# nie-lang/StabStitch2

Hardware: AMD Instinct MI355X
Metric: stitched frames/sec, 720p 2-view (StabStitch++ inference hot path) (higher is better)
Workload: dtype f32; 1 GPU; configs[2]: 720x1280 2-view, 32-frame clip per step per GPU, 7-frame SmoothWarp sliding window, warp NORMAL / fusion AVERAGE, synthetic checkpoints; parallelism=streams1

## Files before the change

__graft_entry__.py:

```python
import os
import subprocess
import sys

ROOT = os.path.dirname(os.path.abspath(__file__))
if ROOT not in sys.path:
    sys.path.insert(0, ROOT)


def build():
    subprocess.run(['bash', os.path.join(ROOT, 'stabstitch2_amd', 'csrc', 'build.sh')], check=True)
    subprocess.run(['bash', os.path.join(ROOT, 'stabstitch2_amd', 'csrc', 'build.sh'), 'tuning'], check=True)
    import re
    from stabstitch2_amd import _hip
    lib = _hip.lib()
    hdr = open(os.path.join(ROOT, 'include', 'stabstitch_hip.h')).read()
    declared = sorted(set(re.findall(r'\b(ss_[a-z0-9_]+)\s*\(', hdr)))
    missing = [n for n in declared if not hasattr(lib, n)]
    if missing:
        raise RuntimeError('libstabstitch_hip.so lacks symbols declared in the header: %s' % missing)
    if sorted(_hip.SIGNATURES) != declared:
        raise RuntimeError('ctypes table and header disagree: %s' % sorted(set(_hip.SIGNATURES) ^ set(declared)))
    from stabstitch2_amd import _blend
    blib = _blend.lib()
    bhdr = open(os.path.join(ROOT, 'include', 'stabstitch_blend.h')).read()
    bdeclared = sorted(set(re.findall(r'\bSSB_API[^;]*?\b(ssb_[a-z0-9_]+)\s*\(', bhdr)))
    missing = [n for n in bdeclared if not hasattr(blib, n)]
    if missing:
        raise RuntimeError('libstabstitch_blend.so lacks symbols declared in the header: %s' % missing)
    if sorted(_blend.SIGNATURES) != bdeclared:
        raise RuntimeError('ctypes table and header disagree: %s' % sorted(set(_blend.SIGNATURES) ^ set(bdeclared)))
    from stabstitch2_amd import _seam
    slib = _seam.lib()
    shdr = open(os.path.join(ROOT, 'include', 'stabstitch_seam.h')).read()
    sdeclared = sorted(set(re.findall(r'\bSSM_API[^;]*?\b(ssm_[a-z0-9_]+)\s*\(', shdr)))
    missing = [n for n in sdeclared if not hasattr(slib, n)]
    if missing:
        raise RuntimeError('libstabstitch_seam.so lacks symbols declared in the header: %s' % missing)
    if sorted(_seam.SIGNATURES) != sdeclared:
        raise RuntimeError('ctypes table and header disagree: %s' % sorted(set(_seam.SIGNATURES) ^ set(sdeclared)))
    from stabstitch2_amd import _mbwarp
    wlib = _mbwarp.lib()
    whdr = open(os.path.join(ROOT, 'include', 'stabstitch_mbwarp.h')).read()
    wdeclared = sorted(set(re.findall(r'\bSSW_API[^;]*?\b(ssw_[a-z0-9_]+)\s*\(', whdr)))
    missing = [n for n in wdeclared if not hasattr(wlib, n)]
    if missing:
        raise RuntimeError('libstabstitch_mbwarp.so lacks symbols declared in the header: %s' % missing)
    if sorted(_mbwarp.SIGNATURES) != wdeclared:
        raise RuntimeError('ctypes table and header disagree: %s' % sorted(set(_mbwarp.SIGNATURES) ^ set(wdeclared)))
    import stabstitch2_amd.pipeline
    print('build ok: four libraries, %d + %d + %d + %d entry points, version %d, blend version %d, seam version %d, mbwarp version %d'
          % (len(declared), len(bdeclared), len(sdeclared), len(wdeclared), lib.ss_version(), blib.ssb_version(), slib.ssm_version(),
             wlib.ssw_version()))


def smoke():
    import numpy as np
    import torch
    from stabstitch2_amd import synth, pipeline, _hip
    from stabstitch2_amd.spatial_network import SpatialNet
    from stabstitch2_amd.temporal_network import TemporalNet
    from stabstitch2_amd.smooth_network import SmoothNet
    from oracle import nets as ON, pipeline as OP
    assert torch.cuda.is_available(), 'smoke() needs cuda:0'
    _hip.lib()
    dev = torch.device('cuda:0')
    torch.set_grad_enabled(False)
    torch.set_num_threads(max(1, min(16, os.cpu_count() or 1)))
    hr, lr = synth.make_clip(7, 360, 480, seed=1)
    hip_nets, cpu_nets = [], []
    for hcls, ocls in ((SpatialNet, ON.SpatialNet), (TemporalNet, ON.TemporalNet), (SmoothNet, ON.SmoothNet)):
        m = hcls()
        sd = synth.synthetic_state_dict(m)
        m.load_state_dict(sd, strict=True)
        hip_nets.append(m.to(dev))
        o = ocls().eval()
        o.load_state_dict(sd, strict=True)
        cpu_nets.append(o)
    frames, hc, wc, m1, m2 = pipeline.run_two_view(hr[0], hr[1], lr[0], lr[1], hip_nets)
    torch.cuda.synchronize()
    oframes, ohc, owc, om1, om2 = OP.run_two_view(hr[0], hr[1], lr[0], lr[1], cpu_nets)
    dm = max(float((m1.cpu() - om1).abs().max()), float((m2.cpu() - om2).abs().max()))
    assert dm < 5e-3, 'mesh mismatch vs oracle: %.4f px' % dm
    assert (hc, wc) == (ohc, owc), ((hc, wc), (ohc, owc))
    got = frames.permute(0, 2, 3, 1).cpu().numpy()
    df = max(float(np.median(np.abs(got[i] - oframes[i]))) for i in range(len(oframes)))
    q = max(float(np.quantile(np.abs(got[i] - oframes[i]), 0.999)) for i in range(len(oframes)))
    assert df < 0.01 and q < 0.5, 'frame mismatch vs oracle: median %.4f, p99.9 %.4f' % (df, q)
    print('smoke ok: canvas %dx%d, mesh max|diff| %.2e px, frame median|diff| %.2e p99.9 %.2e' % (hc, wc, dm, df, q))


if __name__ == '__main__':
    build()
    if len(sys.argv) > 1 and sys.argv[1] == 'smoke':
        smoke()
```

stabstitch2_amd/csrc/conv.hip:

```cpp
#include "common.h"

typedef float f32x16 __attribute__((ext_vector_type(16)));
typedef float f32x4 __attribute__((ext_vector_type(4)));
typedef unsigned u32x4 __attribute__((ext_vector_type(4)));

struct ConvP {
    const float* in;
    const float* wgt;
    const float* bias;
    const float* res;
    float* out;
    float* partial;
    int T, H, W, C;
    int px_b, row_b;
    int To, Ho, Wo, Co;
    int kt, kh, kw, s;
    int pt, ph, pw;
    int K, M;
    SsFastDiv divC, divKw, divKh;
    SsDiv32 divWo, divHo, divTo;
    SsDiv32 divNt, divSplits;
    int relu, out_cs;
    int pool2;
    int splits, tiles_per_split;
    unsigned ntiles;
    long long in_gs, w_gs, out_gs;
    unsigned in_bytes, w_bytes;
#ifdef SS_TUNING
    unsigned long long* dbg;
    int ablate;
#endif
};

#ifdef SS_TUNING
#define SS_ABLATE(p, bit) ((p).ablate & (bit))
#define SS_STAMP(p, var) do { if ((p).dbg) var = __builtin_amdgcn_s_memtime(); } while (0)
#else
#define SS_ABLATE(p, bit) 0
#define SS_STAMP(p, var) do { } while (0)
#endif


__device__ __forceinline__ __amdgpu_buffer_rsrc_t uniform_rsrc(const float* base, unsigned bytes) {
    unsigned long long a = (unsigned long long)base;
    unsigned lo = __builtin_amdgcn_readfirstlane((unsigned)a);
    unsigned hi = __builtin_amdgcn_readfirstlane((unsigned)(a >> 32));
    void* ub = (void*)(((unsigned long long)hi << 32) | lo);
    return __builtin_amdgcn_make_buffer_rsrc(ub, 0, (int)__builtin_amdgcn_readfirstlane(bytes), 0x00020000);
}

template <int WGM, int WGN, int WM, int WN, int NBUF, int MINW = 1, int BK = 32, bool TAIL = false, int SCHED = 0,
          int AMODE = 0>
__global__ __launch_bounds__(256, MINW) void conv_igemm_kernel(ConvP p) {
    constexpr int BM = WGM * WM * 32;
    constexpr int BN = WGN * WN * 32;
    constexpr int LDK = BK + 4;
    constexpr int TPR = BK / 4;
    constexpr int RPP = 256 / TPR;
    constexpr int RA = BM / RPP;
    constexpr int RB = BN / RPP;
    constexpr int NCH = BK / 8;
    __shared__ __attribute__((aligned(16))) float As[NBUF][BM * LDK];
    __shared__ __attribute__((aligned(16))) float Bs[NBUF][BN * LDK];
    extern __shared__ __attribute__((aligned(16))) uint2 tap_tab[];

    const int tid = threadIdx.x;
    const int lane = tid & 63;
    const int wave = tid >> 6;
    const int wr = wave / WGN, wc = wave % WGN;
    int mt, nt;
    {
        const unsigned nwg = gridDim.x, b = blockIdx.x;
        unsigned lin = b;
        if (!SS_ABLATE(p, 8) && nwg >= 16) {
            const unsigned q = nwg / 8, r = nwg % 8, xcd = b % 8, idx = b / 8;
            lin = (xcd < r ? xcd * (q + 1) : r * (q + 1) + (xcd - r) * q) + idx;
        }
        mt = (int)ss_div32(lin, p.divNt);
        nt = (int)(lin - (unsigned)mt * p.ntiles);
    }
    if (!SS_ABLATE(p, 32)) __builtin_amdgcn_s_setprio(3);
#ifdef SS_TUNING
    unsigned long long ts0 = 0, ts1 = 0, ts2 = 0, tsa = 0, tsb = 0, tsc = 0;
#endif
    SS_STAMP(p, ts0);
    const int m0 = mt * BM;
    const int n0 = nt * BN;
    const int grp = (int)ss_div32(blockIdx.z, p.divSplits);
    const int split = blockIdx.z - grp * p.splits;

    const __amdgpu_buffer_rsrc_t rin = uniform_rsrc(p.in + (long long)grp * p.in_gs, p.in_bytes);
    const __amdgpu_buffer_rsrc_t rw = uniform_rsrc(p.wgt + (long long)grp * p.w_gs, p.w_bytes);

    const int lrow = tid / TPR;
    const int kq = tid % TPR;

    __shared__ uint4 rowinfo[BM];
    if (tid < BM) {
        const int m = m0 + tid;
        const bool ok = m < p.M;
        const uint32_t mm = ok ? (uint32_t)m : 0u;
        const uint32_t t1 = ss_div32(mm, p.divWo);
        const int wo = (int)(mm - t1 * (uint32_t)p.Wo);
        const uint32_t t2 = ss_div32(t1, p.divHo);
        const int ho = (int)(t1 - t2 * (uint32_t)p.Ho);
        const uint32_t n = ss_div32(t2, p.divTo);
        const int to = (int)(t2 - n * (uint32_t)p.To);
        const int ti0 = to - p.pt, hi0 = ho * p.s - p.ph, wi0 = wo * p.s - p.pw;
        const int aoff = (((int)n * p.T + ti0) * p.H + hi0) * p.row_b + wi0 * p.px_b;
        auto span = [](int x0, int k, int size) -> unsigned {
            int lo = max(0, -x0), hi = min(k, size - x0);
            return hi > lo ? (1u << hi) - (1u << lo) : 0u;
        };
        unsigned msk = span(wi0, p.kw, p.W) | (span(hi0, p.kh, p.H) << 8) | (span(ti0, p.kt, p.T) << 16);
        msk = ok ? msk : 0u;
        unsigned inv_lo = 0xFFFFFFFFu, inv_hi = 0xFFFFFFFFu;
        if (AMODE == 1 || AMODE == 3) {
            unsigned valid = 0u;
            const unsigned mw = msk & 0xFFu;
            if (p.kw == 1 && p.kt == 1) {
                valid = (mw & (msk >> 16) & 1u) ? ((msk >> 8) & 0xFFu) : 0u;
            } else {
                for (int dt = 0; dt < p.kt; ++dt)
                    for (int dh = 0; dh < p.kh; ++dh) {
                        const unsigned sel = 0u - ((msk >> (8 + dh)) & (msk >> (16 + dt)) & 1u);
                        valid |= (mw << ((dt * p.kh + dh) * p.kw)) & sel;
                    }
            }
            inv_lo = ~valid;
        } else if (AMODE == 2) {
            unsigned long long valid = 0ull;
            const unsigned long long mw = msk & 0xFFu;
            for (int dt = 0; dt < p.kt; ++dt)
// ... 226 lines not shown
        d[5] = tsa; d[6] = tsb; d[7] = tsc;
        d[0] = ts0; d[1] = ts1; d[2] = ts2; d[3] = __builtin_amdgcn_s_memtime();
        d[4] = __builtin_amdgcn_s_getreg((31 << 11) | 4) | ((unsigned long long)__builtin_amdgcn_s_getreg((31 << 11) | 20) << 32);
    }
#endif
}

__global__ void splitk_reduce_kernel(ConvP p) {
    long long idx = (long long)blockIdx.x * blockDim.x + threadIdx.x;
    long long per = (long long)p.M * p.Co;
    int grp = blockIdx.y;
    if (p.pool2) {
        const int hp = p.Ho >> 1, wp = p.Wo >> 1;
        const long long nimg = (long long)p.M / ((long long)p.Ho * p.Wo);
        const long long pper = nimg * hp * wp * p.Co;
        if (idx >= pper) return;
        const int co = (int)(idx % p.Co);
        long long q = idx / p.Co;
        const int x = (int)(q % wp); q /= wp;
        const int y = (int)(q % hp);
        const long long n = q / hp;
        const float* part = p.partial + (long long)grp * p.splits * per;
        const long long m00 = (n * p.Ho + 2 * y) * p.Wo + 2 * x;
        const float* pq = part + m00 * p.Co + co;
        const long long rowo = (long long)p.Wo * p.Co;
        float v[4] = {0.f, 0.f, 0.f, 0.f};
        for (int s0 = 0; s0 < p.splits; s0 += 8) {
            float t[8][4];
#pragma unroll
            for (int k = 0; k < 8; ++k) {
                const bool ok = s0 + k < p.splits;
                const float* qs = pq + (long long)(ok ? s0 + k : s0) * per;
                t[k][0] = ok ? qs[0] : 0.f;
                t[k][1] = ok ? qs[p.Co] : 0.f;
                t[k][2] = ok ? qs[rowo] : 0.f;
                t[k][3] = ok ? qs[rowo + p.Co] : 0.f;
            }
#pragma unroll
            for (int k = 0; k < 8; ++k)
                if (s0 + k < p.splits) {
#pragma unroll
                    for (int i = 0; i < 4; ++i) v[i] += t[k][i];
                }
        }
        float best = fmaxf(fmaxf(v[0], v[1]), fmaxf(v[2], v[3]));
        if (p.bias) best += p.bias[(long long)grp * p.Co + co];
        if (p.relu) best = fmaxf(best, 0.f);
        p.out[(long long)grp * p.out_gs + ((n * hp + y) * wp + x) * p.out_cs + co] = best;
        return;
    }
    if (idx >= per) return;
    int co = (int)(idx % p.Co);
    long long m = idx / p.Co;
    const float* part = p.partial + (long long)grp * p.splits * per + idx;
    float v = 0.f;
    for (int s0 = 0; s0 < p.splits; s0 += 8) {
        float t[8];
#pragma unroll
        for (int k = 0; k < 8; ++k) t[k] = s0 + k < p.splits ? part[(long long)(s0 + k) * per] : 0.f;
#pragma unroll
        for (int k = 0; k < 8; ++k)
            if (s0 + k < p.splits) v += t[k];
    }
    if (p.bias) v += p.bias[(long long)grp * p.Co + co];
    long long o = (long long)grp * p.out_gs + m * p.out_cs + co;
    if (p.res) v += p.res[o];
    if (p.relu) v = fmaxf(v, 0.f);
    p.out[o] = v;
}

#ifdef SS_TUNING
static int g_lds_pad = 0;
static int g_amode_off = 0;
static int g_force_tile = 0;
static int g_ablate = 0;
static int g_split_target = 512;
unsigned long long* ss_tuning_dbg = nullptr;
extern int g_wino_nb1_max_cin, g_wino_ablate, g_wino_variant;
extern int g_stem_kernel;
#define g_dbg ss_tuning_dbg
extern "C" SS_API void ss_debug_ptr(void* ptr) { g_dbg = (unsigned long long*)ptr; }
extern "C" SS_API void ss_debug_set(int key, int value) {
    if (key == 0) g_force_tile = value;
    if (key == 1) g_ablate = value;
    if (key == 2) g_split_target = value;
    if (key == 3) g_amode_off = value;
    if (key == 4) g_lds_pad = value;
    if (key == 5) g_wino_nb1_max_cin = value;
    if (key == 6) g_wino_ablate = value;
    if (key == 7) g_wino_variant = value;
    if (key == 18) g_stem_kernel = value;
}
#else
constexpr int g_lds_pad = 0, g_amode_off = 0, g_force_tile = 0;
constexpr int g_split_target = 512;
#endif

template <int WGM, int WGN, int WM, int WN, int NBUF, int MINW = 1, int BK = 32, bool TAIL = false, int SCHED = 0,
          int AMODE = 0>
static void launch_conv(const ConvP& p, int groups, hipStream_t st, unsigned dyn_lds = 0) {
    constexpr int BM = WGM * WM * 32, BN = WGN * WN * 32;
    ConvP q = p;
    q.ntiles = (unsigned)ss_cdiv(p.Co, BN);
    q.divNt = ss_div32_make(q.ntiles);
    q.divSplits = ss_div32_make((uint32_t)p.splits);
    dim3 g((unsigned)ss_cdiv(p.M, BM) * q.ntiles, 1, groups * p.splits);
    hipLaunchKernelGGL((conv_igemm_kernel<WGM, WGN, WM, WN, NBUF, MINW, BK, TAIL, SCHED, AMODE>), g, dim3(256),
                       dyn_lds + (unsigned)g_lds_pad, st, q);
}

template <int WGM, int WGN, int WM, int WN, int NBUF, int BK = 32, int SCHED = 0>
static void launch_auto(const ConvP& p, int groups, hipStream_t st, int taps, bool tail) {
    const unsigned tab_bytes = (unsigned)p.tiles_per_split * (unsigned)(BK / 4) * 8u;
    constexpr int BN_ = WGN * WN * 32;
    int amode = ((g_amode_off & 1) || taps > 64 || tab_bytes > 24576u) ? 0 : (taps <= 32 ? 1 : 2);
    if (amode == 1 && !(g_amode_off & 2) && p.Co % BN_ == 0 && p.K % BK == 0) amode = 3;
    constexpr bool DEF = WGM == 2 && WGN == 2 && (WM == 1 || WM == 2) && WN == 1 && NBUF == 1 && BK == 32 && SCHED == 1;
    if (DEF && tail) {
        if (amode == 1) launch_conv<WGM, WGN, WM, WN, NBUF, 1, BK, DEF, SCHED, 1>(p, groups, st, tab_bytes);
        else if (amode == 2) launch_conv<WGM, WGN, WM, WN, NBUF, 1, BK, DEF, SCHED, 2>(p, groups, st, tab_bytes);
        else launch_conv<WGM, WGN, WM, WN, NBUF, 1, BK, DEF, SCHED, 0>(p, groups, st);
    } else {
        if (amode == 3) launch_conv<WGM, WGN, WM, WN, NBUF, 1, BK, false, SCHED, 3>(p, groups, st, tab_bytes);
        else if (amode == 1) launch_conv<WGM, WGN, WM, WN, NBUF, 1, BK, false, SCHED, 1>(p, groups, st, tab_bytes);
        else if (amode == 2) launch_conv<WGM, WGN, WM, WN, NBUF, 1, BK, false, SCHED, 2>(p, groups, st, tab_bytes);
        else launch_conv<WGM, WGN, WM, WN, NBUF, 1, BK, false, SCHED, 0>(p, groups, st);
    }
}

static int conv_splits(long long M, int cout, int groups, int nk) {
    long long b64 = (long long)ss_cdiv(M, 64) * ss_cdiv(cout, 64) * groups;
    int want = (int)((g_split_target + b64 - 1) / b64);
    if (want == 2 && nk < 32 && b64 * 5 >= (long long)g_split_target * 3) want = 1;
    int maxs = nk / 4 > 0 ? nk / 4 : 1;
    int splits = want < maxs ? want : maxs;
    if (splits <= 1) return 1;
    const int tps = ss_cdiv(nk, splits);
    return ss_cdiv(nk, tps);
}

extern "C" long long ss_conv_workspace_need(int n, int t, int h, int w, int cin, int cout, int kt, int kh, int kw,
                                            int stride, int pad_t, int pad_h, int pad_w, int groups) {
    if (n <= 0 || t <= 0 || h <= 0 || w <= 0 || cin <= 0 || cout <= 0 || kt <= 0 || kh <= 0 || kw <= 0 || stride <= 0 ||
        groups <= 0)
        return 0;
    const int To = t + 2 * pad_t - kt + 1, Ho = (h + 2 * pad_h - kh) / stride + 1, Wo = (w + 2 * pad_w - kw) / stride + 1;
    if (To <= 0 || Ho <= 0 || Wo <= 0) return 0;
    const long long M = (long long)n * To * Ho * Wo, K = (long long)kt * kh * kw * cin;
    const int splits = conv_splits(M, cout, groups, ss_cdiv(K, 32));
    return splits > 1 ? (long long)groups * splits * M * cout : 0;
}

static int conv_dispatch(ConvP& p, long long K, long long M, int groups, int taps, float* ws, long long ws_floats,
                         hipStream_t st);

extern "C" int ss_conv_nhwc(const float* in, const float* wgt, const float* bias, const float* res, float* out,
                            int n, int t, int h, int w, int cin, int cout, int kt, int kh, int kw, int stride,
                            int pad_t, int pad_h, int pad_w, int relu, int out_cs, int groups, long long in_gs,
                            long long w_gs, long long out_gs, float* ws, long long ws_floats, void* stream) {
    if (!in || !wgt || !out || n <= 0 || t <= 0 || h <= 0 || w <= 0 || cin <= 0 || (cin & 3) || cout <= 0 ||
        kt <= 0 || kh <= 0 || kw <= 0 || kt > 8 || kh > 8 || kw > 8 || stride <= 0 || groups <= 0 || out_cs < cout)
        return SS_ERR_ARG;
    ConvP p;
    p.in = in; p.wgt = wgt; p.bias = bias; p.res = res; p.out = out; p.partial = nullptr;
    p.T = t; p.H = h; p.W = w; p.C = cin;
    p.To = t + 2 * pad_t - kt + 1;
    p.Ho = (h + 2 * pad_h - kh) / stride + 1;
    p.Wo = (w + 2 * pad_w - kw) / stride + 1;
    p.Co = cout;
    if (p.To <= 0 || p.Ho <= 0 || p.Wo <= 0) return SS_ERR_ARG;
    p.kt = kt; p.kh = kh; p.kw = kw; p.s = stride; p.pt = pad_t; p.ph = pad_h; p.pw = pad_w;
    long long K = (long long)kt * kh * kw * cin;
    long long M = (long long)n * p.To * p.Ho * p.Wo;
    long long in_elems = (long long)n * t * h * w * cin;
    long long w_elems = (long long)cout * K;
    if (K >= 65536 || M >= (1ll << 31) || in_elems * 4 >= (1ll << 31) || w_elems * 4 >= (1ll << 31) ||
        M * (long long)(out_cs > cout ? out_cs : cout) * 4 >= (1ll << 32))
        return SS_ERR_UNSUPPORTED;
    p.px_b = cin * 4;
    p.row_b = w * cin * 4;
    p.in_gs = in_gs; p.w_gs = w_gs; p.out_gs = out_gs;
    p.in_bytes = (unsigned)(in_elems * 4);
    p.w_bytes = (unsigned)(w_elems * 4);
    p.relu = relu; p.out_cs = out_cs; p.pool2 = 0;
    return conv_dispatch(p, K, M, groups, kt * kh * kw, ws, ws_floats, (hipStream_t)stream);
}

extern "C" int ss_conv_pool2_nhwc(const float* in, const float* wgt, const float* bias, float* out, int n, int h, int w,
                                  int cin, int cout, int kh, int kw, int stride, int pad_h, int pad_w, int relu, int out_cs,
                                  int groups, long long in_gs, long long w_gs, long long out_gs, float* ws, long long ws_floats,
                                  void* stream) {
    if (!in || !wgt || !out || n <= 0 || h <= 0 || w <= 0 || cin <= 0 || (cin & 3) || cout <= 0 || kh <= 0 || kw <= 0 ||
        kh > 8 || kw > 8 || stride <= 0 || groups <= 0 || out_cs < cout)
// ... 346 lines not shown
    const long long total = (long long)n * h * (w + 8);
    hipLaunchKernelGGL(nchw_to_nhwc3_padded_kernel, dim3(ss_cdiv(total, 256)), dim3(256), 0, (hipStream_t)stream, in, out, h,
                       w, total);
    return ss_launch_status();
}

__global__ void nhwc_to_nchw_kernel(const float* __restrict__ in, float* __restrict__ out, int n, int c, int h, int w,
                                    int cs) {
    long long idx = (long long)blockIdx.x * blockDim.x + threadIdx.x;
    long long hw = (long long)h * w;
    long long total = (long long)n * c * hw;
    if (idx >= total) return;
    long long rem = idx % hw;
    long long bc = idx / hw;
    int ch = (int)(bc % c);
    int b = (int)(bc / c);
    out[idx] = in[((long long)b * hw + rem) * cs + ch];
}

extern "C" int ss_nchw_to_nhwc(const float* in, float* out, int n, int c, int h, int w, int c_pad, void* stream) {
    if (!in || !out || n <= 0 || c <= 0 || h <= 0 || w <= 0 || c_pad < c) return SS_ERR_ARG;
    long long total = (long long)n * h * w * c_pad;
    if (c_pad == 4 && (((uintptr_t)out) & 15) == 0) {
        long long pixels = (long long)n * h * w;
        hipLaunchKernelGGL(nchw_to_nhwc4_kernel, dim3(ss_cdiv(pixels, 256)), dim3(256), 0, (hipStream_t)stream, in,
                           reinterpret_cast<float4*>(out), c, h * w, pixels);
        return ss_launch_status();
    }
    hipLaunchKernelGGL(nchw_to_nhwc_kernel, dim3(ss_cdiv(total, 256)), dim3(256), 0, (hipStream_t)stream, in, out, n, c,
                       h, w, c_pad);
    return ss_launch_status();
}

extern "C" int ss_nhwc_to_nchw(const float* in, float* out, int n, int c, int h, int w, int c_stride, void* stream) {
    if (!in || !out || n <= 0 || c <= 0 || h <= 0 || w <= 0 || c_stride < c) return SS_ERR_ARG;
    long long total = (long long)n * c * h * w;
    hipLaunchKernelGGL(nhwc_to_nchw_kernel, dim3(ss_cdiv(total, 256)), dim3(256), 0, (hipStream_t)stream, in, out, n, c,
                       h, w, c_stride);
    return ss_launch_status();
}

extern "C" int ss_version(void) { return 600; }

extern "C" const char* ss_error_string(int code) {
    switch (code) {
        case SS_OK: return "ok";
        case SS_ERR_ARG: return "bad argument";
        case SS_ERR_LAUNCH: return "kernel launch failed";
        case SS_ERR_UNSUPPORTED: return "unsupported size";
        case SS_ERR_DEVICE: return "kernel not available on this device";
        default: return "unknown error";
    }
}
```

stabstitch2_amd/ops.py:

```python
import collections
import os
import threading

import ctypes

import torch

from . import _hip as H


def _f(t):
    return t if (t.dtype == torch.float32 and t.is_contiguous()) else t.contiguous().float()


class _Built:
    __slots__ = ('value', 'stream', 'event', 'tag')

    def __init__(self, build, device, what, tag=None):
        if torch.cuda.is_current_stream_capturing():
            raise RuntimeError('stabstitch2_amd: %s would be built inside a HIP-graph capture; run the path once eagerly '
                               '(warm-up) before capturing' % what)
        self.value = build()
        self.stream = torch.cuda.current_stream(device)
        self.event = torch.cuda.Event()
# ... 288 lines not shown
    if out is None:
        out = torch.empty(((g, n, h, w, cout) if grouped else (n, h, w, cout)), device=x.device, dtype=torch.float32)
    pk = wino_packed(wgt, g, sliced)
    H.call('ss_conv3x3_wino3_nhwc' if sliced else 'ss_conv3x3_wino_nhwc', H.dptr(x), H.dptr(pk), H.dptr(bias, True), H.dptr(res, True), H.dptr(out),
           n, h, w, cin, cout, int(relu), out.shape[-1], g, in_gs,
           pk.shape[1], out[0].numel() if grouped else 0, H.stream())
    return out


def pool2_is_fused(x, wgt, stride=1, pad=(0, 1, 1)):
    cout, kt, kh, kw, cin = wgt.shape[-5:]
    groups = wgt.shape[0] if wgt.dim() == 6 else 1
    n, h, w = x.shape[-4], x.shape[-3], x.shape[-2]
    return bool(POOL_FUSED and WINO_MATH != 'bf16x9' and _uses_winograd(kt, kh, kw, stride, pad, cin, cout, h, w, n * groups))


POOL_SPLITK = os.environ.get('SS_POOL_SPLITK', '1') == '1'


def pool2_in_reduce(x, wgt, stride=1, pad=(0, 1, 1)):
    cout, kt, kh, kw, cin = wgt.shape[-5:]
    groups = wgt.shape[0] if wgt.dim() == 6 else 1
    n, h, w, c = x.shape[-4:]
    return bool(POOL_SPLITK and kt == 1 and pad[0] == 0 and
                _conv_ws_need(n, 1, h, w, c, cout, 1, kh, kw, stride, 0, pad[1], pad[2], groups) > 0)


def _conv_pool2_splitk(x, wgt, bias, stride, pad, relu, groups):
    if not POOL_SPLITK:
        return None
    grouped = wgt.dim() == 6
    cout, kt, kh, kw, cin = wgt.shape[-5:]
    n, h, w, c = x.shape[-4:]
    pt, ph, pw = pad
    if kt != 1 or pt != 0:
        return None
    need = _conv_ws_need(n, 1, h, w, c, cout, 1, kh, kw, stride, 0, ph, pw, groups)
    if need <= 0:
        return None
    ho = (h + 2 * ph - kh) // stride + 1
    wo = (w + 2 * pw - kw) // stride + 1
    shape = (groups, n, ho // 2, wo // 2, cout) if grouped else (n, ho // 2, wo // 2, cout)
    out = torch.empty(shape, device=x.device, dtype=torch.float32)
    ws = conv_workspace(x.device, need)
    shared = grouped and x.dim() == 4
    global last_conv_path
    last_conv_path = 'igemm'
    H.call('ss_conv_pool2_nhwc', H.dptr(x), H.dptr(wgt), H.dptr(bias, True), H.dptr(out), n, h, w, c, cout, kh, kw, stride, ph, pw,
           int(relu), cout, groups, 0 if (shared or not grouped) else x[0].numel(), wgt[0].numel() if grouped else 0,
           out[0].numel() if grouped else 0, H.dptr(ws), ws.numel(), H.stream())
    return out


def conv(x, wgt, bias=None, res=None, stride=1, pad=(0, 1, 1), relu=False, out=None, pool2=False):
    if pool2:
        assert x.dim() == 4 and out is None and res is None
        if pool2_is_fused(x, wgt, stride, pad):
            return conv_winograd(x, wgt, bias, None, relu, None, pool2=True)
        y = _conv_pool2_splitk(x, wgt, bias, stride, pad, relu, 1)
        return y if y is not None else maxpool(conv(x, wgt, bias, None, stride, pad, relu), 2, 2, 0)
    five = x.dim() == 5
    if five:
        n, t, h, w, c = x.shape
    else:
        n, h, w, c = x.shape
        t = 1
    cout, kt, kh, kw, cin = wgt.shape
    assert cin == c, (cin, c)
    pt, ph, pw = pad
    to = t + 2 * pt - kt + 1
    ho = (h + 2 * ph - kh) // stride + 1
    wo = (w + 2 * pw - kw) // stride + 1
    if out is None:
        shape = (n, to, ho, wo, cout) if five else (n, ho, wo, cout)
        out = torch.empty(shape, device=x.device, dtype=torch.float32)
    if not five and _uses_wino43(kt, kh, kw, stride, pad, c, cout, ho, wo, n):
        y = _try_wino43(x, wgt, bias, res, relu, out)
        if y is not None:
            return y
    if not five and _uses_winograd(kt, kh, kw, stride, pad, c, cout, ho, wo, n):
        return conv_winograd(x, wgt, bias, res, relu, out)
    global last_conv_path
    last_conv_path = 'igemm'
    ws = conv_workspace(x.device, _conv_ws_need(n, t, h, w, c, cout, kt, kh, kw, stride, pt, ph, pw, 1))
    H.call('ss_conv_nhwc', H.dptr(x), H.dptr(wgt), H.dptr(bias, True), H.dptr(res, True), H.dptr(out),
           n, t, h, w, c, cout, kt, kh, kw, stride, pt, ph, pw, int(relu), out.shape[-1],
           1, 0, 0, 0, H.dptr(ws, True), 0 if ws is None else ws.numel(), H.stream())
    return out


def conv_grouped(x, wgt, bias=None, res=None, stride=1, pad=(0, 1, 1), relu=False, pool2=False, out=None):
    g2, cout, kt, kh, kw, cin = wgt.shape
    shared = x.dim() == 4
    if shared:
        n, h, w, c = x.shape
        g = g2
    else:
        g, n, h, w, c = x.shape
    assert g2 == g and cin == c and kt == 1, (wgt.shape, x.shape)
    pt, ph, pw = pad
    ho = (h + 2 * ph - kh) // stride + 1
    wo = (w + 2 * pw - kw) // stride + 1
    if pool2:
        assert res is None and out is None
        if pool2_is_fused(x, wgt, stride, pad):
            return conv_winograd(x, wgt, bias, None, relu, None, pool2=True)
        y = _conv_pool2_splitk(x, wgt, bias, stride, pad, relu, g)
        if y is not None:
            return y
        y = conv_grouped(x, wgt, bias, None, stride, pad, relu)
        return maxpool(y.view(g * n, ho, wo, cout), 2, 2, 0).view(g, n, ho // 2, wo // 2, cout)
    if out is None:
        out = torch.empty((g, n, ho, wo, cout), device=x.device, dtype=torch.float32)
    assert tuple(out.shape) == (g, n, ho, wo, cout) and out.is_contiguous()
    if _uses_wino43(kt, kh, kw, stride, pad, c, cout, ho, wo, n, g):
        y = _try_wino43(x, wgt, bias, res, relu, out)
        if y is not None:
            return y
    if _uses_winograd(kt, kh, kw, stride, pad, c, cout, ho, wo, n * g):
        return conv_winograd(x, wgt, bias, res, relu, out)
    global last_conv_path
    last_conv_path = 'igemm'
    ws = conv_workspace(x.device, _conv_ws_need(n, 1, h, w, c, cout, kt, kh, kw, stride, pt, ph, pw, g))
    H.call('ss_conv_nhwc', H.dptr(x), H.dptr(wgt), H.dptr(bias, True), H.dptr(res, True), H.dptr(out),
           n, 1, h, w, c, cout, kt, kh, kw, stride, pt, ph, pw, int(relu), cout,
           g, 0 if shared else x[0].numel(), wgt[0].numel(), out[0].numel(), H.dptr(ws, True),
           0 if ws is None else ws.numel(), H.stream())
    return out


def maxpool(x, k, stride, pad=0, out=None):
    n, h, w, c = x.shape
    ho = (h + 2 * pad - k) // stride + 1
    wo = (w + 2 * pad - k) // stride + 1
    if out is None:
        out = torch.empty((n, ho, wo, c), device=x.device, dtype=torch.float32)
    H.call('ss_maxpool_nhwc', H.dptr(x), H.dptr(out), n, h, w, c, k, stride, pad, H.stream())
# ... 1057 lines not shown
```

stabstitch2_amd/pipeline.py:

```python
import glob
import os

import torch

from . import grid_res, ops
from .spatial_network import get_rigid_mesh, get_norm_mesh, build_SpatialNet

grid_h = grid_res.GRID_H
grid_w = grid_res.GRID_W
LR_H, LR_W = 360, 480
WINDOW = 7


def recover_mesh(norm_mesh, height, width):
    b = norm_mesh.size()[0]
    x = (norm_mesh[..., 0] + 1) * float(width) / 2.
    y = (norm_mesh[..., 1] + 1) * float(height) / 2.
    return torch.stack([x, y], 2).reshape([b, grid_h + 1, grid_w + 1, 2])


def linear_blender(ref, tgt, ref_m, tgt_m, mask=False):
    if mask:
        return ops.linear_blend(None, None, ref_m[0, 0].contiguous(), tgt_m[0, 0].contiguous(), True)[None, None]
    return ops.linear_blend(ref[0].contiguous(), tgt[0].contiguous(), ref_m[0, 0].contiguous(),
# ... 174 lines not shown
        if cache1 is None:
            f64_1, f32_1, f64_2, f32_2 = f64[:b], f32[:b], f64[b:], f32[b:]
        else:
            (f64_1, f32_1), f64_2, f32_2 = cache1, f64, f32
        off1, off_ref, off_tgt = self.spatial_net.forward_pair(f64_1, f64_2, f32_1, f32_2, LR_H, LR_W)
        if self.cache2 is not None:
            self.cache2.append((f64_2, f32_2))
        ops.spatial_meshes(off1, off_ref, off_tgt, LR_H, LR_W, out=(self.m1[s:e], self.m2[s:e]))

    def _temporal(self, xb, b, s, e):
        L, tp = self.L, self.tp
        nv = len(self.views)
        f = L.run_trunk_body(xb, tp['s1'])
        lead = 0 if s == 0 else 1
        rows = b - 1 + lead
        if rows > 0:
            cv = torch.empty((nv * rows, f.shape[1], f.shape[2], 52), device=f.device, dtype=torch.float32)
            slices = []
            for i in range(nv):
                fi = f[i * b:(i + 1) * b]
                if lead:
                    ops.cost_volume(self.carry[i], fi[0:1], 3, out=cv[i * rows:i * rows + 1])
                if b > 1:
                    ops.cost_volume(fi[:b - 1], fi[1:], 3, out=cv[i * rows + lead:(i + 1) * rows])
                slices.append((i * rows, (i + 1) * rows, self.tm[i, e - rows:e].view(rows, -1)))
            L.run_regressor(cv, tp['r2'], out_slices=slices)
        self._carry(f, b, nv, e)

    def result(self):
        if self.pos != self.n:
            raise ValueError('%d of %d frames pushed' % (self.pos, self.n))
        self.carry = None
        if self.tmotion1 is not None:
            return self.m1, self.m2, self.tmotion1, self.tm[0]
        return self.m1, self.m2, self.tm[0], self.tm[1]


@torch.no_grad()
def joint_stage(spatial_net, temporal_net, lr1, lr2, chunk=None, tmotion1=None, cache2=None, cache1=None):
    chunk = chunk or SPATIAL_CHUNK
    n = lr2.shape[0]
    est = JointEstimator(spatial_net, temporal_net, n, lr2.device, tmotion1, cache2)
    for i, s in enumerate(range(0, n, chunk)):
        est.push(None if cache1 is not None else lr1[s:s + chunk], lr2[s:s + chunk], None if cache1 is None else cache1[i])
    return est.result()


@torch.no_grad()
def smooth_stage(smooth_net, s1, s2, t1, t2):
    n = s1.shape[0]
    smesh1, tsm1 = ops.tsmotion(s1, t1, LR_H, LR_W)
    smesh2, tsm2 = ops.tsmotion(s2, t2, LR_H, LR_W)
    nw = n - (WINDOW - 1)
    delta = smooth_net.window_deltas(smesh1, smesh2, tsm1, tsm2, nw, WINDOW, 1, 1)
    out = ops.smooth_stitch(smesh1, smesh2, tsm1, tsm2, delta, nw, WINDOW)
    out['smotion1'], out['smotion2'], out['tmotion1'], out['tmotion2'] = s1, s2, t1, t2
    out['tsmotion1'], out['tsmotion2'] = tsm1, tsm2
    return out


@torch.no_grad()
def estimate_meshes(nets, lr1, lr2, tmotion1=None, spatial_cache1=None, keep_spatial_cache2=False):
    spatial_net, temporal_net, smooth_net = nets
    dev = next(spatial_net.parameters()).device
    if isinstance(lr1, (list, tuple)):
        lr1 = torch.cat([t.to(dev) for t in lr1], 0)
        lr2 = torch.cat([t.to(dev) for t in lr2], 0)
    n = lr1.shape[0]
    if n < WINDOW:
        raise ValueError('need at least %d frames for the sliding smooth window, got %d' % (WINDOW, n))
    cache2 = [] if keep_spatial_cache2 else None
    if OVERLAP_STREAMS:
        main = torch.cuda.current_stream(dev)
        side = _side_stream(dev)
        side.wait_stream(main)
        with torch.cuda.stream(side):
            t1, t2 = temporal_stage_views(temporal_net, [lr1, lr2])
        s1, s2 = spatial_stage(spatial_net, lr1, lr2)
        main.wait_stream(side)
        for t in (t1, t2):
            t.record_stream(main)
    elif SHARED_STEM and (tmotion1 is None) == (spatial_cache1 is None):
        s1, s2, t1, t2 = joint_stage(spatial_net, temporal_net, lr1, lr2, tmotion1=tmotion1, cache2=cache2, cache1=spatial_cache1)
    else:
        s1, s2 = spatial_stage(spatial_net, lr1, lr2, cache1=spatial_cache1)
        if tmotion1 is None:
            t1, t2 = temporal_stage_views(temporal_net, [lr1, lr2])
        else:
            t1, t2 = tmotion1, temporal_stage_views(temporal_net, [lr2])[0]
    out = smooth_stage(smooth_net, s1, s2, t1, t2)
    if cache2:
        out['spatial_cache2'] = cache2
    return out


def _stitch_windows(o):
    out = {}
    for k in ('ori_mesh1', 'ori_mesh2', 'smooth_mesh1', 'smooth_mesh2'):
        out[k] = torch.cat((o[k][0], o[k][1:, -1]), 0).unsqueeze(0)
    op, sp = o['ori_path2'], o['smooth_path2']
    inc = op[1:, -1] - op[1:, -2]
    ori_path = torch.cat((op[0], op[0, -1:] + torch.cumsum(inc, 0)), 0)
    smooth_path = torch.cat((sp[0], ori_path[WINDOW:] + (sp[1:, -1] - op[1:, -1])), 0)
    out['ori_path2'] = ori_path.unsqueeze(0)
    out['smooth_path2'] = smooth_path.unsqueeze(0)
    return out

# ... 690 lines not shown
```

stabstitch2_amd/smooth_network.py:

```python
import torch
import torch.nn as nn

from . import grid_res, layers as L, ops

grid_h = grid_res.GRID_H
grid_w = grid_res.GRID_W
WINDOW_CHUNK = 2048


class MotionPrediction(nn.Module):

    def __init__(self, kernel=5):
        super().__init__()
        self.embedding1 = nn.Sequential(nn.Linear(2, 32), nn.ReLU())
        self.embedding2 = nn.Sequential(nn.Linear(1, 8), nn.ReLU())
        self.embedding3 = nn.Sequential(nn.Linear(2, 32), nn.ReLU())
        self.pad = kernel // 2
        self.MotionConv3D = nn.Sequential(
            nn.Conv3d(128, 128, (kernel, 3, 3), padding=(self.pad, 1, 1)), nn.ReLU(),
            nn.Conv3d(128, 128, (kernel, 3, 3), padding=(self.pad, 1, 1)), nn.ReLU(),
            nn.Conv3d(128, 128, (kernel, 3, 3), padding=(self.pad, 1, 1)), nn.ReLU())
        self.decoding = nn.Sequential(nn.Linear(128, 4))


class SmoothNet(L.PreparedMixin, nn.Module):
    def __init__(self, dropout=0.):
        super().__init__()
        self.MotionPre = MotionPrediction()
        self.eval()

    def _prepare(self):
        mp = self.MotionPre
        return {'e1': L.pack_fc(mp.embedding1[0]), 'e3': L.pack_fc(mp.embedding3[0]),
                'conv': [L.pack_conv3d(mp.MotionConv3D[i]) for i in (0, 2, 4)], 'pad': mp.pad,
                'dec': L.pack_fc(mp.decoding[0])}

    @torch.no_grad()
    def window_deltas(self, smesh1, smesh2, ts1, ts2, nw, t, wstride, zero_first, out=None):
        p = self._prepared()
        if out is None:
            out = torch.empty((nw, t, grid_h + 1, grid_w + 1, 4), device=smesh1.device, dtype=torch.float32)
        if nw > WINDOW_CHUNK and wstride <= t:
            for s in range(0, nw, WINDOW_CHUNK):
                m = min(WINDOW_CHUNK, nw - s)
                f0, f1 = s * wstride, (s + m - 1) * wstride + t
                self.window_deltas(smesh1[f0:f1], smesh2[f0:f1], ts1[f0:f1], ts2[f0:f1], m, t, wstride, zero_first, out[s:s + m])
            return out
        hid = ops.smooth_embed(smesh1, smesh2, ts1, ts2, p['e1'][0], p['e1'][1], p['e3'][0], p['e3'][1], nw, t,
                               wstride, zero_first)
        for w, b in p['conv']:
            hid = ops.conv(hid, w, b, stride=1, pad=(p['pad'], 1, 1), relu=True)
        ops.linear(hid.view(-1, 128), p['dec'][0], p['dec'][1], out=out.view(-1, 4))
        return out

    @torch.no_grad()
    def run_windows(self, smesh1, smesh2, ts1, ts2, nw, t, wstride, zero_first):
        delta = self.window_deltas(smesh1, smesh2, ts1, ts2, nw, t, wstride, zero_first)
        out = ops.smooth_finalize(smesh1, smesh2, ts1, ts2, delta.view(-1, 4), nw, t, wstride, zero_first)
        return out, delta

    def forward(self, smesh_list1, smesh_list2, tsmotion_list1, tsmotion_list2):
        dev = next(self.parameters()).device
        t = len(smesh_list1)
        st = [torch.stack([x.to(dev).float() for x in lst], 1).contiguous()
              for lst in (smesh_list1, smesh_list2, tsmotion_list1, tsmotion_list2)]
        b = st[0].shape[0]
        flat = [x.view(b * t, grid_h + 1, grid_w + 1, 2) for x in st]
        o, delta = self.run_windows(flat[0], flat[1], flat[2], flat[3], b, t, t, 0)
        return (o['ori_mesh1'], o['ori_mesh2'], o['ori_path1'], o['ori_path2'], delta[..., 0:2], delta[..., 2:4])


@torch.no_grad()
def build_SmoothNet(net, tsmotion_list1, tsmotion_list2, smesh_list1, smesh_list2):
    dev = next(net.parameters()).device
    t = len(smesh_list1)
    st = [torch.stack([x.to(dev).float() for x in lst], 1).contiguous()
          for lst in (smesh_list1, smesh_list2, tsmotion_list1, tsmotion_list2)]
    b = st[0].shape[0]
    flat = [x.view(b * t, grid_h + 1, grid_w + 1, 2) for x in st]
    return net.run_windows(flat[0], flat[1], flat[2], flat[3], b, t, t, 0)[0]
```

Baseline: 4363 frames/s.

## Skip SmoothNet conv output tiles outside the receptive field of kept frames

Adds a conv variant that takes a keep range (the first window computed in full, later windows only from a given output frame on) and returns early for GEMM tiles and split-K reduce rows whose frames fall outside it. The sliding-window smoothing only needs the last frame of most windows, so each Conv3D layer computes only the frames inside that frame's temporal receptive field, shrinking as layers get deeper. This removes redundant Conv3D work across overlapping windows. The skipped outputs stay uninitialized, so correctness relies on downstream code reading only the last frame of those windows. It also adds a separate library and a limited set of tile configurations.

```diff
diff --git a/__graft_entry__.py b/__graft_entry__.py
--- a/__graft_entry__.py
+++ b/__graft_entry__.py
@@ -47,22 +47,33 @@
         raise RuntimeError('libstabstitch_mbwarp.so lacks symbols declared in the header: %s' % missing)
     if sorted(_mbwarp.SIGNATURES) != wdeclared:
         raise RuntimeError('ctypes table and header disagree: %s' % sorted(set(_mbwarp.SIGNATURES) ^ set(wdeclared)))
+    from stabstitch2_amd import _convkeep
+    klib = _convkeep.lib()
+    khdr = open(os.path.join(ROOT, 'include', 'stabstitch_convkeep.h')).read()
+    kdeclared = sorted(set(re.findall(r'\bSSK_API[^;]*?\b(ssk_[a-z0-9_]+)\s*\(', khdr)))
+    missing = [n for n in kdeclared if not hasattr(klib, n)]
+    if missing:
+        raise RuntimeError('libstabstitch_convkeep.so lacks symbols declared in the header: %s' % missing)
+    if sorted(_convkeep.SIGNATURES) != kdeclared:
+        raise RuntimeError('ctypes table and header disagree: %s' % sorted(set(_convkeep.SIGNATURES) ^ set(kdeclared)))
     import stabstitch2_amd.pipeline
-    print('build ok: four libraries, %d + %d + %d + %d entry points, version %d, blend version %d, seam version %d, mbwarp version %d'
-          % (len(declared), len(bdeclared), len(sdeclared), len(wdeclared), lib.ss_version(), blib.ssb_version(), slib.ssm_version(),
-             wlib.ssw_version()))
+    print('build ok: five libraries, %d + %d + %d + %d + %d entry points, version %d, blend version %d, seam version %d, '
+          'mbwarp version %d, convkeep version %d'
+          % (len(declared), len(bdeclared), len(sdeclared), len(wdeclared), len(kdeclared), lib.ss_version(), blib.ssb_version(),
+             slib.ssm_version(), wlib.ssw_version(), klib.ssk_version()))
 
 
 def smoke():
     import numpy as np
     import torch
-    from stabstitch2_amd import synth, pipeline, _hip
+    from stabstitch2_amd import synth, pipeline, _hip, _convkeep
     from stabstitch2_amd.spatial_network import SpatialNet
     from stabstitch2_amd.temporal_network import TemporalNet
     from stabstitch2_amd.smooth_network import SmoothNet
     from oracle import nets as ON, pipeline as OP
     assert torch.cuda.is_available(), 'smoke() needs cuda:0'
     _hip.lib()
+    _convkeep.lib()
     dev = torch.device('cuda:0')
     torch.set_grad_enabled(False)
     torch.set_num_threads(max(1, min(16, os.cpu_count() or 1)))
diff --git a/include/stabstitch_convkeep.h b/include/stabstitch_convkeep.h
--- /dev/null
+++ b/include/stabstitch_convkeep.h
@@ -0,0 +1,31 @@
+#ifndef STABSTITCH_CONVKEEP_H
+#define STABSTITCH_CONVKEEP_H
+
+#ifdef __cplusplus
+extern "C" {
+#endif
+
+#if defined(_WIN32)
+#define SSK_API __declspec(dllexport)
+#else
+#define SSK_API __attribute__((visibility("default")))
+#endif
+
+#define SSK_OK 0
+#define SSK_ERR_ARG -1
+#define SSK_ERR_LAUNCH -2
+#define SSK_ERR_UNSUPPORTED -3
+
+SSK_API int ssk_version(void);
+
+SSK_API long long ssk_conv_keep_workspace_need(int n, int t, int h, int w, int cin, int cout, int kt, int kh, int kw, int stride,
+                                               int pad_t, int pad_h, int pad_w);
+
+SSK_API int ssk_conv_keep_nhwc(const float* in, const float* wgt, const float* bias, float* out, int n, int t, int h, int w, int cin,
+                               int cout, int kt, int kh, int kw, int stride, int pad_t, int pad_h, int pad_w, int relu, int out_cs,
+                               int full_items, int keep_from, float* ws, long long ws_floats, void* stream);
+
+#ifdef __cplusplus
+}
+#endif
+#endif
diff --git a/stabstitch2_amd/_convkeep.py b/stabstitch2_amd/_convkeep.py
--- /dev/null
+++ b/stabstitch2_amd/_convkeep.py
@@ -0,0 +1,65 @@
+import ctypes
+import os
+
+import torch
+
+from . import _hip as H
+
+LIB_PATH = os.path.join(os.path.dirname(os.path.abspath(__file__)), 'libstabstitch_convkeep.so')
+ERR_ARG = -1
+ERR_UNSUPPORTED = -3
+
+c_fp, c_i, c_ll, c_st = H.c_fp, H.c_i, H.c_ll, H.c_st
+
+SIGNATURES = {
+    'ssk_version': (c_i, []),
+    'ssk_conv_keep_workspace_need': (c_ll, [c_i] * 13),
+    'ssk_conv_keep_nhwc': (c_i, [c_fp] * 4 + [c_i] * 17 + [c_fp, c_ll, c_st]),
+}
+
+_lib = None
+
+
+def lib():
+    global _lib
+    if _lib is None:
+        if not os.path.exists(LIB_PATH):
+            raise ImportError(
+                'stabstitch2_amd: %s not found. Build it with `python -c "import __graft_entry__ as g; g.build()"` '
+                'or stabstitch2_amd/csrc/build.sh (hipcc --offload-arch=gfx950). There is no CPU fallback.' % LIB_PATH)
+        handle = ctypes.CDLL(LIB_PATH)
+        for name, (res, args) in SIGNATURES.items():
+            fn = getattr(handle, name)
+            fn.restype = res
+            fn.argtypes = args
+        _lib = handle
+    return _lib
+
+
+def call(name, *args):
+    dev = None
+    for a in args:
+        d = getattr(a, 'dev', None)
+        if d is not None:
+            if dev is not None and d != dev:
+                raise H.HipError('%s: tensors of one launch live on different GPUs (cuda:%d and cuda:%d)' % (name, dev, d))
+            dev = d
+    if dev is None:
+        raise H.HipError('%s needs device tensors; there is no CPU path' % name)
+    st = ctypes.c_void_p(torch.cuda.current_stream(dev).cuda_stream)
+    args = tuple(st if a is H._STREAM else a for a in args)
+    fn = getattr(lib(), name)
+    if dev == torch.cuda.current_device():
+        code = fn(*args)
+    else:
+        with torch.cuda.device(dev):
+            code = fn(*args)
+    if code == ERR_UNSUPPORTED:
+        return False
+    if code == ERR_ARG:
+        raise ValueError('%s refused its arguments' % name)
+    if code != 0:
+        err = H.HipError('%s failed: launch error (%d)' % (name, code))
+        err.code = code
+        raise err
+    return True
diff --git a/stabstitch2_amd/csrc/conv.hip b/stabstitch2_amd/csrc/conv.hip
--- a/stabstitch2_amd/csrc/conv.hip
+++ b/stabstitch2_amd/csrc/conv.hip
@@ -26,6 +26,9 @@
     unsigned ntiles;
     long long in_gs, w_gs, out_gs;
     unsigned in_bytes, w_bytes;
+#ifdef SS_CONV_KEEP
+    int keep_full, keep_from;
+#endif
 #ifdef SS_TUNING
     unsigned long long* dbg;
     int ablate;
@@ -48,6 +51,25 @@
     void* ub = (void*)(((unsigned long long)hi << 32) | lo);
     return __builtin_amdgcn_make_buffer_rsrc(ub, 0, (int)__builtin_amdgcn_readfirstlane(bytes), 0x00020000);
 }
+
+#ifdef SS_CONV_KEEP
+__device__ __forceinline__ void conv_keep_frame(const ConvP& p, uint32_t m, uint32_t& n, uint32_t& to) {
+    const uint32_t t2 = ss_div32(ss_div32(m, p.divWo), p.divHo);
+    n = ss_div32(t2, p.divTo);
+    to = t2 - n * (uint32_t)p.To;
+}
+__device__ __forceinline__ bool conv_keep_row(const ConvP& p, uint32_t m) {
+    uint32_t n, to;
+    conv_keep_frame(p, m, n, to);
+    return (int)n < p.keep_full || (int)to >= p.keep_from;
+}
+__device__ __forceinline__ bool conv_keep_tile(const ConvP& p, int m0, int bm) {
+    uint32_t n0, to0, n1, to1;
+    conv_keep_frame(p, (uint32_t)m0, n0, to0);
+    conv_keep_frame(p, (uint32_t)(min(m0 + bm, p.M) - 1), n1, to1);
+    return (int)n0 < p.keep_full || n1 != n0 || (int)to1 >= p.keep_from;
+}
+#endif
 
 template <int WGM, int WGN, int WM, int WN, int NBUF, int MINW = 1, int BK = 32, bool TAIL = false, int SCHED = 0,
           int AMODE = 0>
@@ -79,6 +101,9 @@
         mt = (int)ss_div32(lin, p.divNt);
         nt = (int)(lin - (unsigned)mt * p.ntiles);
     }
+#ifdef SS_CONV_KEEP
+    if (!conv_keep_tile(p, mt * BM, BM)) return;
+#endif
     if (!SS_ABLATE(p, 32)) __builtin_amdgcn_s_setprio(3);
 #ifdef SS_TUNING
     unsigned long long ts0 = 0, ts1 = 0, ts2 = 0, tsa = 0, tsb = 0, tsc = 0;
@@ -411,6 +436,9 @@
     if (idx >= per) return;
     int co = (int)(idx % p.Co);
     long long m = idx / p.Co;
+#ifdef SS_CONV_KEEP
+    if (!conv_keep_row(p, (uint32_t)m)) return;
+#endif
     const float* part = p.partial + (long long)grp * p.splits * per + idx;
     float v = 0.f;
     for (int s0 = 0; s0 < p.splits; s0 += 8) {
@@ -498,6 +526,7 @@
     return ss_cdiv(nk, tps);
 }
 
+#ifndef SS_CONV_KEEP
 extern "C" long long ss_conv_workspace_need(int n, int t, int h, int w, int cin, int cout, int kt, int kh, int kw,
                                             int stride, int pad_t, int pad_h, int pad_w, int groups) {
     if (n <= 0 || t <= 0 || h <= 0 || w <= 0 || cin <= 0 || cout <= 0 || kt <= 0 || kh <= 0 || kw <= 0 || stride <= 0 ||
@@ -950,3 +979,4 @@
         default: return "unknown error";
     }
 }
+#endif
diff --git a/stabstitch2_amd/csrc/convkeep.hip b/stabstitch2_amd/csrc/convkeep.hip
--- /dev/null
+++ b/stabstitch2_amd/csrc/convkeep.hip
@@ -0,0 +1,96 @@
+#define SS_CONV_KEEP 1
+#include "conv.hip"
+
+#include "../../include/stabstitch_convkeep.h"
+
+static_assert(SSK_OK == SS_OK && SSK_ERR_ARG == SS_ERR_ARG && SSK_ERR_LAUNCH == SS_ERR_LAUNCH &&
+              SSK_ERR_UNSUPPORTED == SS_ERR_UNSUPPORTED, "the error codes are the main library's");
+
+static int keep_plan(ConvP& p, long long K, long long M, int taps, float* ws, long long ws_floats) {
+    const int cout = p.Co;
+    const int nk = ss_cdiv(K, 32);
+    p.splits = 1;
+    p.tiles_per_split = nk;
+    p.partial = nullptr;
+    const bool tail = (K % 32) != 0 && (K % 32) < 16;
+    const int splits = conv_splits(M, cout, 1, nk);
+    const long long need = (long long)splits * M * cout;
+    if (splits > 1 && ws && need <= ws_floats && need < (1ll << 31)) {
+        p.tiles_per_split = ss_cdiv(nk, splits);
+        p.splits = ss_cdiv(nk, p.tiles_per_split);
+        p.partial = ws;
+    }
+    const unsigned tab_bytes = (unsigned)p.tiles_per_split * 8u * 8u;
+    if (tail || taps <= 32 || taps > 64 || tab_bytes > 24576u) return 0;
+    const long long b128 = (long long)ss_cdiv(M, 64) * (cout / 128);
+    const long long b128m = (long long)ss_cdiv(M, 128) * ss_cdiv(cout, 64);
+    if (p.splits == 1 && cout % 128 == 0 && b128 >= 2048) return 128;
+    if (p.splits == 1 && b128m >= 2048) return 0;
+    return 64;
+}
+
+static bool keep_geometry(int n, int t, int h, int w, int cin, int cout, int kt, int kh, int kw, int stride, int pad_t, int pad_h,
+                          int pad_w, int& To, int& Ho, int& Wo) {
+    if (n <= 0 || t <= 0 || h <= 0 || w <= 0 || cin <= 0 || (cin & 3) || cout <= 0 || kt <= 0 || kh <= 0 || kw <= 0 || kt > 8 ||
+        kh > 8 || kw > 8 || stride <= 0 || pad_t < 0 || pad_h < 0 || pad_w < 0)
+        return false;
+    To = t + 2 * pad_t - kt + 1;
+    Ho = (h + 2 * pad_h - kh) / stride + 1;
+    Wo = (w + 2 * pad_w - kw) / stride + 1;
+    return To > 0 && Ho > 0 && Wo > 0;
+}
+
+extern "C" int ssk_version(void) { return 1; }
+
+extern "C" long long ssk_conv_keep_workspace_need(int n, int t, int h, int w, int cin, int cout, int kt, int kh, int kw, int stride,
+                                                  int pad_t, int pad_h, int pad_w) {
+    int To, Ho, Wo;
+    if (!keep_geometry(n, t, h, w, cin, cout, kt, kh, kw, stride, pad_t, pad_h, pad_w, To, Ho, Wo)) return 0;
+    const long long M = (long long)n * To * Ho * Wo, K = (long long)kt * kh * kw * cin;
+    const int splits = conv_splits(M, cout, 1, ss_cdiv(K, 32));
+    return splits > 1 ? (long long)splits * M * cout : 0;
+}
+
+extern "C" int ssk_conv_keep_nhwc(const float* in, const float* wgt, const float* bias, float* out, int n, int t, int h, int w,
+                                  int cin, int cout, int kt, int kh, int kw, int stride, int pad_t, int pad_h, int pad_w, int relu,
+                                  int out_cs, int full_items, int keep_from, float* ws, long long ws_floats, void* stream) {
+    ConvP p;
+    if (!in || !wgt || !out || out_cs < cout ||
+        !keep_geometry(n, t, h, w, cin, cout, kt, kh, kw, stride, pad_t, pad_h, pad_w, p.To, p.Ho, p.Wo))
+        return SS_ERR_ARG;
+    if (full_items < 0 || full_items > n || keep_from < 0 || keep_from >= p.To) return SS_ERR_ARG;
+    const long long K = (long long)kt * kh * kw * cin;
+    const long long M = (long long)n * p.To * p.Ho * p.Wo;
+    const long long in_elems = (long long)n * t * h * w * cin;
+    const long long w_elems = (long long)cout * K;
+    if (K >= 65536 || M >= (1ll << 31) || in_elems * 4 >= (1ll << 31) || w_elems * 4 >= (1ll << 31) ||
+        M * (long long)out_cs * 4 >= (1ll << 32))
+        return SS_ERR_ARG;
+    p.in = in; p.wgt = wgt; p.bias = bias; p.res = nullptr; p.out = out;
+    p.T = t; p.H = h; p.W = w; p.C = cin;
+    p.Co = cout;
+    p.kt = kt; p.kh = kh; p.kw = kw; p.s = stride; p.pt = pad_t; p.ph = pad_h; p.pw = pad_w;
+    p.px_b = cin * 4;
+    p.row_b = w * cin * 4;
+    p.in_gs = 0; p.w_gs = 0; p.out_gs = 0;
+    p.in_bytes = (unsigned)(in_elems * 4);
+    p.w_bytes = (unsigned)(w_elems * 4);
+    p.relu = relu; p.out_cs = out_cs; p.pool2 = 0;
+    p.K = (int)K; p.M = (int)M;
+    p.divC = ss_fastdiv_make((uint32_t)cin);
+    p.divKw = ss_fastdiv_make((uint32_t)kw);
+    p.divKh = ss_fastdiv_make((uint32_t)kh);
+    p.divWo = ss_div32_make((uint32_t)p.Wo);
+    p.divHo = ss_div32_make((uint32_t)p.Ho);
+    p.divTo = ss_div32_make((uint32_t)p.To);
+    p.keep_full = full_items; p.keep_from = keep_from;
+    const int tile = keep_plan(p, K, M, kt * kh * kw, ws, ws_floats);
+    if (!tile) return SS_ERR_UNSUPPORTED;
+    hipStream_t st = (hipStream_t)stream;
+    const unsigned tab_bytes = (unsigned)p.tiles_per_split * 8u * 8u;
+    if (tile == 128) launch_conv<2, 2, 1, 2, 1, 1, 32, false, 1, 2>(p, 1, st, tab_bytes);
+    else launch_conv<2, 2, 1, 1, 1, 1, 32, false, 1, 2>(p, 1, st, tab_bytes);
+    if (p.splits > 1)
+        hipLaunchKernelGGL(splitk_reduce_kernel, dim3(ss_cdiv(M * cout, 256), 1), dim3(256), 0, st, p);
+    return ss_launch_status();
+}
diff --git a/stabstitch2_amd/ops.py b/stabstitch2_amd/ops.py
--- a/stabstitch2_amd/ops.py
+++ b/stabstitch2_amd/ops.py
@@ -364,7 +364,9 @@
     return out
 
 
-def conv(x, wgt, bias=None, res=None, stride=1, pad=(0, 1, 1), relu=False, out=None, pool2=False):
+def conv(x, wgt, bias=None, res=None, stride=1, pad=(0, 1, 1), relu=False, out=None, pool2=False, keep=None):
+    if keep is not None and (pool2 or res is not None):
+        raise ValueError('conv: keep= goes with neither pool2 nor a residual')
     if pool2:
         assert x.dim() == 4 and out is None and res is None
         if pool2_is_fused(x, wgt, stride, pad):
@@ -395,6 +397,14 @@
     global last_conv_path
     last_conv_path = 'igemm'
     ws = conv_workspace(x.device, _conv_ws_need(n, t, h, w, c, cout, kt, kh, kw, stride, pt, ph, pw, 1))
+    if keep is not None:
+        from . import _convkeep as K
+        full_items, keep_from = keep
+        if K.call('ssk_conv_keep_nhwc', H.dptr(x), H.dptr(wgt), H.dptr(bias, True), H.dptr(out), n, t, h, w, c, cout, kt, kh, kw,
+                  stride, pt, ph, pw, int(relu), out.shape[-1], int(full_items), int(keep_from), H.dptr(ws, True),
+                  0 if ws is None else ws.numel(), H.stream()):
+            last_conv_path = 'igemm-keep'
+            return out
     H.call('ss_conv_nhwc', H.dptr(x), H.dptr(wgt), H.dptr(bias, True), H.dptr(res, True), H.dptr(out),
            n, t, h, w, c, cout, kt, kh, kw, stride, pt, ph, pw, int(relu), out.shape[-1],
            1, 0, 0, 0, H.dptr(ws, True), 0 if ws is None else ws.numel(), H.stream())
diff --git a/stabstitch2_amd/pipeline.py b/stabstitch2_amd/pipeline.py
--- a/stabstitch2_amd/pipeline.py
+++ b/stabstitch2_amd/pipeline.py
@@ -250,7 +250,7 @@
     smesh1, tsm1 = ops.tsmotion(s1, t1, LR_H, LR_W)
     smesh2, tsm2 = ops.tsmotion(s2, t2, LR_H, LR_W)
     nw = n - (WINDOW - 1)
-    delta = smooth_net.window_deltas(smesh1, smesh2, tsm1, tsm2, nw, WINDOW, 1, 1)
+    delta = smooth_net.window_deltas(smesh1, smesh2, tsm1, tsm2, nw, WINDOW, 1, 1, keep_last=nw > 1)
     out = ops.smooth_stitch(smesh1, smesh2, tsm1, tsm2, delta, nw, WINDOW)
     out['smotion1'], out['smotion2'], out['tmotion1'], out['tmotion2'] = s1, s2, t1, t2
     out['tsmotion1'], out['tsmotion2'] = tsm1, tsm2
diff --git a/stabstitch2_amd/smooth_network.py b/stabstitch2_amd/smooth_network.py
--- a/stabstitch2_amd/smooth_network.py
+++ b/stabstitch2_amd/smooth_network.py
@@ -36,7 +36,7 @@
                 'dec': L.pack_fc(mp.decoding[0])}
 
     @torch.no_grad()
-    def window_deltas(self, smesh1, smesh2, ts1, ts2, nw, t, wstride, zero_first, out=None):
+    def window_deltas(self, smesh1, smesh2, ts1, ts2, nw, t, wstride, zero_first, out=None, keep_last=False, _first=True):
         p = self._prepared()
         if out is None:
             out = torch.empty((nw, t, grid_h + 1, grid_w + 1, 4), device=smesh1.device, dtype=torch.float32)
@@ -44,12 +44,15 @@
             for s in range(0, nw, WINDOW_CHUNK):
                 m = min(WINDOW_CHUNK, nw - s)
                 f0, f1 = s * wstride, (s + m - 1) * wstride + t
-                self.window_deltas(smesh1[f0:f1], smesh2[f0:f1], ts1[f0:f1], ts2[f0:f1], m, t, wstride, zero_first, out[s:s + m])
+                self.window_deltas(smesh1[f0:f1], smesh2[f0:f1], ts1[f0:f1], ts2[f0:f1], m, t, wstride, zero_first, out[s:s + m],
+                                   keep_last, s == 0)
             return out
         hid = ops.smooth_embed(smesh1, smesh2, ts1, ts2, p['e1'][0], p['e1'][1], p['e3'][0], p['e3'][1], nw, t,
                                wstride, zero_first)
-        for w, b in p['conv']:
-            hid = ops.conv(hid, w, b, stride=1, pad=(p['pad'], 1, 1), relu=True)
+        last = len(p['conv']) - 1
+        for i, (w, b) in enumerate(p['conv']):
+            keep = (1 if _first else 0, max(0, t - 1 - (last - i) * p['pad'])) if keep_last else None
+            hid = ops.conv(hid, w, b, stride=1, pad=(p['pad'], 1, 1), relu=True, keep=keep)
         ops.linear(hid.view(-1, 128), p['dec'][0], p['dec'][1], out=out.view(-1, 4))
         return out
 
```

After: 4354 frames/s. No clear change (-0.2%).
